# Snowdar/asv-subtools

Hardware: NVIDIA H100
Metric: frames/sec x-vector extraction (80-d fbank) (higher is better)
Workload: dtype f32 (bf16x3 split operands on wgmma, fp32 accumulate in registers)

## Files before the change

asv_subtools_b200/csrc/tdnn_gemm.cu:

```cuda
#include <cuda.h>
#include <cuda_bf16.h>
#include <cuda_runtime.h>

#include <stdlib.h>

#include <mutex>

#include "common.cuh"
#include "ptx.cuh"

namespace xvb {

constexpr int kBlockM = 128;
constexpr int kBlockK = 64;
constexpr int kABytes = kBlockM * kBlockK * 2;
constexpr int kNumConsumers = 256;
constexpr int kProducerWarp = kNumConsumers / 32;
constexpr int kSlabBytes = 16384;
constexpr int kStagePlaneBytes = 64 * kBlockK * 2;
constexpr int kStageOutBytes = 2 * kStagePlaneBytes;
constexpr int kCoefBytes = 3 * kBlockK * 4;
constexpr int kEpiBytes = 2 * (kStageOutBytes + kCoefBytes);
static_assert(kEpiBytes >= kSlabBytes, "the histogram slab lives in the epilogue region");

template <int BLOCK_N, bool kHist, bool kSwish>
__host__ __device__ constexpr bool ping_pong() { return BLOCK_N == 128 && !kHist && !kSwish; }
template <int BLOCK_N, bool kHist, bool kSwish>
__host__ __device__ constexpr int gemm_threads() { return kNumConsumers + (ping_pong<BLOCK_N, kHist, kSwish>() ? 128 : 32); }
constexpr uint32_t kProducerRegs = 40, kConsumerRegs = 232;

struct TdnnGemmParams {
  int B, T, Cin, Cout;
  int Tb, Bb, num_t_blk, num_b_blk, num_n_blk, num_tiles;
  int ntaps, cin_p16, num_cblk;
  int ctx[XVB_MAX_TAPS];
  int flags;
  const float* bias;
  const float* scale;
  const float* shift;
  const float* row_bias;
  const float* utt_bias;
  long long ld_utt;
  int log2_tb;
  float* pool_partial;
  int num_src;
  int unit_first, unit_stride;
  unsigned long long* hist;
  const int* row_label;
  const int* col_label;
  float hist_lo, hist_inv_w;
  int hist_bins;
  int hist_sym;
  int hist_group, num_units;
  int k_slices, kb_per_slice;
  int group_ng, group_kg;
  int out_T;
  const int* lengths;
  int tma_store;
#ifdef XVB_TILE_TIMELINE
  unsigned long long* timeline;
  int timeline_tiles;
  int timeline_general;
#endif
  __nv_bfloat16* y_hi;
  __nv_bfloat16* y_lo;
  long long ldy;
  float* y_f32;
  long long ldyf;
};

template <int BLOCK_N, bool kPool, bool kHist>
__host__ __device__ constexpr bool staged_epilogue() { return !kPool && !kHist && BLOCK_N % kBlockK == 0; }

template <int BLOCK_N, bool kPool, bool kHist>
struct GemmCfg {
  static constexpr int kTailBytes = (staged_epilogue<BLOCK_N, kPool, kHist>() || kPool) ? kEpiBytes : kSlabBytes;
  static constexpr int kBBytes = BLOCK_N * kBlockK * 2;
  static constexpr int kStageBytes = 2 * kABytes + 2 * kBBytes;
  static constexpr int kStages = (192 * 1024) / kStageBytes > 6 ? 6 : (192 * 1024) / kStageBytes;
  static constexpr int kAccRegs = BLOCK_N / 2;
  static constexpr int kSmemBytes = kStages * kStageBytes + kTailBytes + 1024  + 256 ;
  static_assert(kSmemBytes <= 232448, "exceeds the 227 KB shared memory of an sm_90 CTA");
  static_assert(kStages >= 2, "need at least a double-buffered operand pipeline");
};

template <bool kHist>
__device__ __forceinline__ bool decode_tile(const TdnnGemmParams& p, int tile, int& m_unit, int& n_blk, int& slice) {
  slice = 0;
  if constexpr (!kHist) {
    if (p.k_slices > 1) { slice = tile % p.k_slices; tile /= p.k_slices; }
    m_unit = p.unit_first + (tile / p.num_n_blk) * p.unit_stride;
    n_blk = tile % p.num_n_blk;
    return true;
  } else {
    const int per_band = p.num_n_blk * p.hist_group;
    const int band = tile / per_band, r = tile - band * per_band;
    n_blk = r / p.hist_group;
    const int mi = band * p.hist_group + (r - n_blk * p.hist_group);
    m_unit = 2 * (p.unit_first + (mi >> 1) * p.unit_stride) + (mi & 1);
    return mi < 2 * p.num_units && !(p.hist_sym && n_blk < m_unit);
  }
}

__device__ __forceinline__ void chan_merge(float& n, float& mean, float& m2, float nb, float meanb, float m2b) {
  const float tot = n + nb;
  if (tot > 0.f) {
    const float d = meanb - mean, wb = nb / tot;
    mean = fmaf(d, wb, mean);
    m2 += m2b + d * d * n * wb;
  }
  n = tot;
}

__device__ __noinline__ float epi_tanh(float v) { return tanhf(v); }
__device__ __noinline__ float epi_sigmoid(float v) { return 1.f / (1.f + expf(-v)); }

__device__ __noinline__ void epi_zero_row(const TdnnGemmParams& p, long long grow, long long frow, int c_begin, int c_end) {
  for (int c = c_begin; c < c_end; c += 8) {
    const bool has1 = c + 1 < p.Cout;
    if (p.y_hi) {
      if (has1) {
        *reinterpret_cast<uint32_t*>(p.y_hi + grow * p.ldy + c) = 0u;
        *reinterpret_cast<uint32_t*>(p.y_lo + grow * p.ldy + c) = 0u;
      } else {
        p.y_hi[grow * p.ldy + c] = __float2bfloat16(0.f);
        p.y_lo[grow * p.ldy + c] = __float2bfloat16(0.f);
      }
    }
    if (p.y_f32) {
      float* df = p.y_f32 + frow * p.ldyf + c;
      if (has1) *reinterpret_cast<float2*>(df) = make_float2(0.f, 0.f);
      else *df = 0.f;
    }
  }
}

#ifdef XVB_TILE_TIMELINE
#define XVB_TL(...) __VA_ARGS__
constexpr int kTimelineHead = 8, kTimelineRec = 12;
static unsigned long long* g_timeline = nullptr;
static int g_timeline_tiles = 0;
static bool g_timeline_direct = false;
__device__ __forceinline__ unsigned long long global_timer() {
  unsigned long long t;
  asm volatile("mov.u64 %0, %%globaltimer;" : "=l"(t));
  return t;
}
#else
#define XVB_TL(...)
#endif

template <int BLOCK_N, bool kPool, bool kHist, bool kSwish = false>
__global__ void __launch_bounds__(gemm_threads<BLOCK_N, kHist, kSwish>(), 1)
tdnn_gemm_bf16x3_kernel(const __grid_constant__ CUtensorMap map_a_hi, const __grid_constant__ CUtensorMap map_a_lo,
                        const __grid_constant__ CUtensorMap map_a2_hi, const __grid_constant__ CUtensorMap map_a2_lo,
                        const __grid_constant__ CUtensorMap map_w_hi, const __grid_constant__ CUtensorMap map_w_lo,
                        const __grid_constant__ CUtensorMap map_y_hi, const __grid_constant__ CUtensorMap map_y_lo,
                        const __grid_constant__ TdnnGemmParams p) {
  constexpr bool kStaged = staged_epilogue<BLOCK_N, kPool, kHist>();
  using Cfg = GemmCfg<BLOCK_N, kPool, kHist>;
  constexpr int kStages = Cfg::kStages;
  constexpr int kBBytes = Cfg::kBBytes;
  constexpr int kStageBytes = Cfg::kStageBytes;
  static_assert(!kPool || BLOCK_N == kBlockM, "fused pooling: 128 channels x 128 frames per tile");
  constexpr bool kPingPong = ping_pong<BLOCK_N, kHist, kSwish>();
  constexpr int kHalves = kPingPong ? 2 : 1;
  constexpr int kReleaseWarps = kPingPong ? 4 : kNumConsumers / 32;

  extern __shared__ uint8_t smem_raw[];
  uint8_t* smem = reinterpret_cast<uint8_t*>((reinterpret_cast<uintptr_t>(smem_raw) + 1023) & ~uintptr_t(1023));
  uint8_t* slab_base = smem + kStages * kStageBytes;
  uint64_t* full_bar = reinterpret_cast<uint64_t*>(slab_base + Cfg::kTailBytes);
  uint64_t* empty_bar = full_bar + kStages;

  const int warp = threadIdx.x >> 5;
  const int lane = threadIdx.x & 31;

  if (warp == kProducerWarp && lane == 0) {
    tma_prefetch_desc(&map_a_hi);
    tma_prefetch_desc(&map_a_lo);
    tma_prefetch_desc(&map_w_hi);
    tma_prefetch_desc(&map_w_lo);
    if ((kStaged || kPool) && p.tma_store) {
      tma_prefetch_desc(&map_y_hi);
      tma_prefetch_desc(&map_y_lo);
    }
    for (int i = 0; i < kStages; ++i) {
      mbar_init(&full_bar[i], 1);
      mbar_init(&empty_bar[i], kReleaseWarps);
    }
    fence_barrier_init();
  }
  __syncthreads();
  asm volatile("griddepcontrol.wait;" ::: "memory");
  asm volatile("fence.proxy.async;" ::: "memory");

  const int num_kblk = p.num_src * p.ntaps * p.num_cblk;

  if (warp >= kProducerWarp) {
    if constexpr (kPingPong) setmaxnreg_dec<kProducerRegs>();
    if (warp == kProducerWarp && lane == 0) {
      int stage = 0;
      uint32_t phase = 0;
      for (int tile = blockIdx.x; tile < p.num_tiles; tile += gridDim.x) {
        int m_unit, n_blk, slice;
        if (!decode_tile<kHist>(p, tile, m_unit, n_blk, slice)) continue;
        const int cb_begin = slice * p.kb_per_slice;
        const int cb_end = p.k_slices > 1 ? min(p.num_cblk, cb_begin + p.kb_per_slice) : p.num_cblk;
        const int b0 = (m_unit / p.num_t_blk) * p.Bb, t0 = (m_unit % p.num_t_blk) * p.Tb;
        const int n0 = n_blk * BLOCK_N;
        const int a_c0 = p.group_ng ? (n0 / p.group_ng) * p.group_kg : 0;
        for (int src = 0; src < p.num_src; ++src) {
          const CUtensorMap* ma_hi = src == 0 ? &map_a_hi : &map_a2_hi;
          const CUtensorMap* ma_lo = src == 0 ? &map_a_lo : &map_a2_lo;
          for (int tap = 0; tap < p.ntaps; ++tap) {
            const int tt = t0 + p.ctx[tap];
            for (int cb = cb_begin; cb < cb_end; ++cb) {
              mbar_wait(&empty_bar[stage], phase ^ 1);
              uint8_t* s = smem + stage * kStageBytes;
              const int kw = tap * p.cin_p16 + cb * kBlockK;
              mbar_expect_tx(&full_bar[stage], kStageBytes);
              tma_load_3d(s, ma_hi, &full_bar[stage], a_c0 + cb * kBlockK, tt, b0);
              tma_load_3d(s + kABytes, ma_lo, &full_bar[stage], a_c0 + cb * kBlockK, tt, b0);
              tma_load_2d(s + 2 * kABytes, &map_w_hi, &full_bar[stage], kw, n0);
              tma_load_2d(s + 2 * kABytes + kBBytes, &map_w_lo, &full_bar[stage], kw, n0);
              if (++stage == kStages) { stage = 0; phase ^= 1; }
            }
          }
        }
      }
    }
    return;
  }

  if constexpr (kPingPong) setmaxnreg_inc<kConsumerRegs>();
  const int wg = warp >> 2;
  const int q4 = lane & 3;
  const int row_base = kPingPong ? 0 : 64 * wg;
  const int row0 = row_base + 16 * (warp & 3) + (lane >> 2);
  const int etid = threadIdx.x;
  const bool relu = (p.flags & XVB_RELU) != 0;
  const bool bn = (p.flags & XVB_BN) != 0;
  const bool act_sigmoid = (p.flags & XVB_SIGMOID) != 0;
  const bool act_tanh = (p.flags & XVB_TANH) != 0;
  const float relu_floor = relu ? 0.f : -INFINITY;
  float acc[kHalves][Cfg::kAccRegs];
#pragma unroll
  for (int hh = 0; hh < kHalves; ++hh)
#pragma unroll
    for (int i = 0; i < Cfg::kAccRegs; ++i) acc[hh][i] = 0.f;
  auto half_down = [&]() {
#pragma unroll
    for (int i = 0; i < Cfg::kAccRegs; ++i) acc[0][i] = acc[kHalves - 1][i];
  };
  int stage = 0;
  uint32_t phase = 0;
  uint32_t it = 0;

  uint32_t h_below[2] = {0u, 0u}, h_above[2] = {0u, 0u};
  const uint32_t hslab = smem_u32(slab_base);
  auto hist_flush = [&]() {
    asm volatile("bar.sync 1, 256;" ::: "memory");
#pragma unroll
    for (int c = 0; c < 2; ++c) {
      if (h_below[c]) asm volatile("red.shared.add.u32 [%0], %1;" ::"r"(hslab + (c * p.hist_bins) * 4), "r"(h_below[c]) : "memory");
      if (h_above[c]) asm volatile("red.shared.add.u32 [%0], %1;" ::"r"(hslab + (c * p.hist_bins + p.hist_bins - 1) * 4), "r"(h_above[c]) : "memory");
      h_below[c] = 0u; h_above[c] = 0u;
    }
    asm volatile("bar.sync 1, 256;" ::: "memory");
    for (int e = etid; e < 2 * p.hist_bins; e += kNumConsumers) {
      uint32_t c;
      asm volatile("ld.shared.u32 %0, [%1];" : "=r"(c) : "r"(hslab + e * 4) : "memory");
      if (c) {
        atomicAdd(p.hist + e, (unsigned long long)c);
        asm volatile("st.shared.u32 [%0], %1;" ::"r"(hslab + e * 4), "r"(0u) : "memory");
      }
    }
    asm volatile("bar.sync 1, 256;" ::: "memory");
  };
  if constexpr (kHist) {
    for (int e = etid; e < 2 * p.hist_bins; e += kNumConsumers)
      asm volatile("st.shared.u32 [%0], %1;" ::"r"(hslab + e * 4), "r"(0u) : "memory");
    asm volatile("bar.sync 1, 256;" ::: "memory");
  }

  XVB_TL(
    long long tl_start = 0, tl_first = 0, tl_issued = 0, tl_retired = 0, tl_wait = 0;
    long long tl_ep[4] = {0, 0, 0, 0};
    long long tl_t = 0;
    auto tl_mark = [&](int ph) { const long long t = clock64(); tl_ep[ph] += t - tl_t; tl_t = t; };
    unsigned long long* tl_cta = p.timeline ? p.timeline + (size_t)blockIdx.x * (kTimelineHead + (size_t)kTimelineRec * p.timeline_tiles) : nullptr;
    if (tl_cta && threadIdx.x == 0) { tl_cta[0] = global_timer(); tl_cta[1] = (unsigned long long)clock64(); }
  )
  int tj = 0;
  XVB_TL(auto tl_flush = [&]() {
    if (tl_cta && (threadIdx.x & 127) == 0 && tj < p.timeline_tiles) {
      unsigned long long* r = tl_cta + kTimelineHead + (size_t)kTimelineRec * tj;
      r[0] = (unsigned long long)tl_start; r[1] = (unsigned long long)tl_first; r[2] = (unsigned long long)tl_issued;
      r[3] = (unsigned long long)tl_retired; r[4] = (unsigned long long)clock64(); r[5] = (unsigned long long)tl_wait;
      r[6] = (unsigned long long)wg; r[7] = 1ull;
      for (int ph = 0; ph < 4; ++ph) r[8 + ph] = (unsigned long long)tl_ep[ph];
    }
  };)
  for (int tile = blockIdx.x; tile < p.num_tiles; tile += gridDim.x, ++tj) {
    int m_unit, n_blk, slice;
    if (!decode_tile<kHist>(p, tile, m_unit, n_blk, slice)) continue;
    int kb_begin = 0, kb_end = num_kblk;
    if (p.k_slices > 1) {
      kb_begin = slice * p.kb_per_slice;
      kb_end = min(num_kblk, kb_begin + p.kb_per_slice);
    }
    if constexpr (kPingPong) {
      if ((tj & 1) != wg) {
        stage += kb_end - kb_begin;
        phase ^= (uint32_t)(stage / kStages) & 1u;
        stage %= kStages;
        continue;
      }
      if (tj > 0) {
        if (kPool && (threadIdx.x & 127) == 0) tma_store_wait_read<0>();
        asm volatile("bar.sync %0, 256;" ::"r"(2 + wg) : "memory");
      }
    }
    ++it;
    XVB_TL(tl_start = clock64(); tl_wait = 0; tl_ep[0] = tl_ep[1] = tl_ep[2] = tl_ep[3] = 0;)
    auto stage_before = [&]() { return stage == 0 ? kStages - 1 : stage - 1; };
    for (int kb = kb_begin; kb < kb_end; ++kb) {
      XVB_TL(const long long tl_w0 = clock64();)
      mbar_wait(&full_bar[stage], phase);
      XVB_TL(const long long tl_w1 = clock64(); tl_wait += tl_w1 - tl_w0; tl_first = kb == kb_begin ? tl_w1 : tl_first;)
      const uint32_t sa = smem_u32(smem + stage * kStageBytes);
      const uint64_t dx_hi = make_sw128_desc(sa), dx_lo = make_sw128_desc(sa + kABytes);
      const uint64_t dw_hi = make_sw128_desc(sa + 2 * kABytes), dw_lo = make_sw128_desc(sa + 2 * kABytes + kBBytes);
      const uint64_t da_hi = kPool ? dw_hi : dx_hi, da_lo = kPool ? dw_lo : dx_lo;
      const uint64_t db_hi = kPool ? dx_hi : dw_hi, db_lo = kPool ? dx_lo : dw_lo;
      wgmma_fence();
#pragma unroll
      for (int s = 0; s < kBlockK / 16; ++s) {
        const uint64_t koff = (uint64_t)(s * 32 >> 4);
#pragma unroll
        for (int hh = 0; hh < kHalves; ++hh) {
          const uint64_t m_off = (uint64_t)((row_base + 64 * hh) * 128 >> 4);
          wgmma_bf16<BLOCK_N>(acc[hh], da_lo + m_off + koff, db_hi + koff, s == 0 ? (uint32_t)(kb != kb_begin) : 1u);
          wgmma_bf16<BLOCK_N>(acc[hh], da_hi + m_off + koff, db_lo + koff, 1);
          wgmma_bf16<BLOCK_N>(acc[hh], da_hi + m_off + koff, db_hi + koff, 1);
        }
      }
      wgmma_commit();
      wgmma_wait<1>();
      if (kb != kb_begin && lane == 0) mbar_arrive(&empty_bar[stage_before()]);
      if (++stage == kStages) { stage = 0; phase ^= 1; }
    }
    if (kPingPong && tile + gridDim.x < p.num_tiles) asm volatile("bar.arrive %0, 256;" ::"r"(3 - wg) : "memory");
    XVB_TL(tl_issued = clock64();)
    wgmma_wait<0>();
    XVB_TL(tl_retired = clock64(); tl_t = tl_retired;)
#pragma unroll
    for (int hh = 0; hh < kHalves; ++hh) wgmma_fence_operands(acc[hh]);
    if (kb_end > kb_begin && lane == 0) mbar_arrive(&empty_bar[stage_before()]);

    const int b0 = (m_unit / p.num_t_blk) * p.Bb, t0 = (m_unit % p.num_t_blk) * p.Tb;
    const int n0 = n_blk * BLOCK_N;

    if constexpr (kPool) {
      int nv = p.T - t0;
      nv = nv < 0 ? 0 : (nv > p.Tb ? p.Tb : nv);
      const int tblk = m_unit % p.num_t_blk;
      const int gl = p.Tb < 8 ? p.Tb : 8;
#pragma unroll 1
      for (int hh = 0; hh < kHalves; ++hh) {
      if (hh > 0) half_down();
      int b0h = b0, nvh = nv;
      asm volatile("" : "+r"(b0h), "+r"(nvh));
      if (p.tma_store && p.Tb == 8 && nvh == 8 XVB_TL(&& !p.timeline_general)) {
#pragma unroll
        for (int h = 0; h < 2; ++h) {
          const int cch = n0 + row0 + 64 * hh + 8 * h;
          const bool cvalid = cch < p.Cout;
          const float bias_c = (cvalid && p.bias) ? __ldg(p.bias + cch) : 0.f;
          const float scale_c = (cvalid && bn) ? __ldg(p.scale + cch) : 1.f;
          const float shift_c = (cvalid && bn) ? __ldg(p.shift + cch) : 0.f;
          int tid = threadIdx.x;
          asm volatile("" : "+r"(tid));
          const uint32_t dst0 = smem_u32(slab_base) + (tid >> 7) * kStageOutBytes +
                                4 * (16 * ((tid >> 5) & 3) + ((tid & 31) >> 2) + 64 * hh + 8 * h);
#pragma unroll
          for (int i = 0; i < BLOCK_N / 8; ++i) {
            const float x0 = fmaf(fmaxf(acc[0][4 * i + 2 * h] + bias_c, relu_floor), scale_c, shift_c);
            const float x1 = fmaf(fmaxf(acc[0][4 * i + 2 * h + 1] + bias_c, relu_floor), scale_c, shift_c);
            float mean = 0.5f * (x0 + x1) + 0.f;
            float m2 = 0.5f * (x0 - x1) * (x0 - x1);
            float d = __shfl_xor_sync(0xffffffffu, mean, 1) - mean;
            float m2b = __shfl_xor_sync(0xffffffffu, m2, 1);
            mean = fmaf(d, 0.5f, mean);
            m2 += m2b + d * d * 2.f * 0.5f;
            d = __shfl_xor_sync(0xffffffffu, mean, 2) - mean;
            m2b = __shfl_xor_sync(0xffffffffu, m2, 2);
            mean = fmaf(d, 0.5f, mean);
            m2 += m2b + d * d * 4.f * 0.5f;
            if (q4 == 0) {
              st_shared_f32(dst0 + 2 * 4 * BLOCK_N * i, mean);
              st_shared_f32(dst0 + 2 * 4 * BLOCK_N * i + 4 * BLOCK_N, m2);
            }
          }
        }
        XVB_TL(tl_mark(2);)
        continue;
      }
#pragma unroll
      for (int h = 0; h < 2; ++h) {
        const int cch = n0 + row0 + 64 * hh + 8 * h;
        const bool cvalid = cch < p.Cout;
        const float bias_c = (cvalid && p.bias) ? __ldg(p.bias + cch) : 0.f;
        const float scale_c = (cvalid && bn) ? __ldg(p.scale + cch) : 1.f;
        const float shift_c = (cvalid && bn) ? __ldg(p.shift + cch) : 0.f;
        auto emit = [&](int col, float mean, float m2) {
          const int bb = b0h + (col >> p.log2_tb);
          if (cvalid && bb < p.B) {
            float* dst = p.pool_partial + ((long long)tblk * p.B + bb) * (2LL * p.Cout) + cch;
            dst[0] = mean;
            dst[p.Cout] = m2;
          }
        };
        float rn = 0.f, rmean = 0.f, rm2 = 0.f;
#pragma unroll
        for (int i = 0; i < BLOCK_N / 8; ++i) {
          const int col = 8 * i + 2 * q4;
          const float x0 = fmaf(fmaxf(acc[0][4 * i + 2 * h] + bias_c, relu_floor), scale_c, shift_c);
          const float x1 = fmaf(fmaxf(acc[0][4 * i + 2 * h + 1] + bias_c, relu_floor), scale_c, shift_c);
          if (p.Tb == 1) {
            if (nvh > 0) { emit(col, x0, 0.f); emit(col + 1, x1, 0.f); }
            continue;
          }
          const int j = col & (p.Tb - 1);
          const bool v0 = j < nvh, v1 = j + 1 < nvh;
          const float pn = (float)v0 + (float)v1;
          const float pm = v1 ? 0.5f * (x0 + x1) : (v0 ? x0 : 0.f);
          const float pm2 = v1 ? 0.5f * (x0 - x1) * (x0 - x1) : 0.f;
          chan_merge(rn, rmean, rm2, pn, pm, pm2);
          if (((col - 2 * q4 + 8) & (p.Tb - 1)) == 0) {
            if (gl >= 4) chan_merge(rn, rmean, rm2, __shfl_xor_sync(0xffffffffu, rn, 1),
                                    __shfl_xor_sync(0xffffffffu, rmean, 1), __shfl_xor_sync(0xffffffffu, rm2, 1));
            if (gl >= 8) chan_merge(rn, rmean, rm2, __shfl_xor_sync(0xffffffffu, rn, 2),
                                    __shfl_xor_sync(0xffffffffu, rmean, 2), __shfl_xor_sync(0xffffffffu, rm2, 2));
            if (((2 * q4) & (gl - 1)) == 0 && rn > 0.f) emit(col & ~(p.Tb - 1), rmean, rm2);
            rn = 0.f; rmean = 0.f; rm2 = 0.f;
          }
        }
      }
      }
      XVB_TL(tl_mark(2);)
      if (p.tma_store && p.Tb == 8 && nv == 8 XVB_TL(&& !p.timeline_general)) {
        fence_proxy_async();
        asm volatile("bar.sync %0, 128;" ::"r"(4 + wg) : "memory");
        XVB_TL(tl_mark(1);)
        if ((threadIdx.x & 127) == 0) {
          tma_store_4d(&map_y_hi, smem_u32(slab_base) + wg * kStageOutBytes, n0, 0, b0, tblk);
          tma_store_commit();
        }
        XVB_TL(tl_mark(3);)
      }
      XVB_TL(tl_flush();)
      continue;
    }

    if constexpr (kHist) {
      const float top = (float)(p.hist_bins - 2);
#pragma unroll
      for (int h = 0; h < 2; ++h) {
        const int row = row0 + 8 * h;
        const int b = b0 + (row >> p.log2_tb), t = t0 + (row & (p.Tb - 1));
        const bool valid = (b < p.B) && (t < p.T);
        const float rbias = (p.row_bias && valid) ? __ldg(p.row_bias + (long long)b * p.T + t) : 0.f;
        const int lab_r = valid ? __ldg(p.row_label + b) : -1;
#pragma unroll
        for (int i = 0; i < BLOCK_N / 8; ++i) {
#pragma unroll
          for (int e = 0; e < 2; ++e) {
            const int c = n0 + 8 * i + 2 * q4 + e;
            const bool in = c < p.Cout;
            const uint32_t ok = (valid && in && (!p.hist_sym || c > b)) ? 1u : 0u;
            const float sc = acc[0][4 * i + 2 * h + e] + ((in && p.bias) ? __ldg(p.bias + c) : 0.f) + rbias;
            const float x = (sc - p.hist_lo) * p.hist_inv_w;
            const uint32_t cls = (in && __ldg(p.col_label + c) == lab_r) ? 1u : 0u;
            const uint32_t bl = x < 0.f ? ok : 0u;
            const uint32_t ab = !(x < top) ? ok : 0u;
            h_below[0] += bl & (cls ^ 1u); h_below[1] += bl & cls;
            h_above[0] += ab & (cls ^ 1u); h_above[1] += ab & cls;
            if (ok & ~(bl | ab))
              asm volatile("red.shared.add.u32 [%0], %1;" ::"r"(hslab + ((int)cls * p.hist_bins + 1 + (int)x) * 4), "r"(1u) : "memory");
          }
        }
      }
      if ((it & 0x3fffu) == 0) hist_flush();
      continue;
    }

    if constexpr (kStaged) {
      if (p.tma_store) {
        int tid = threadIdx.x;
        asm volatile("" : "+r"(tid));
        const int wgo = tid >> 7, wtid = tid & 127, q4o = tid & 3;
        const int prow = 16 * ((tid >> 5) & 3) + ((tid & 31) >> 2);
        const uint32_t stg = smem_u32(slab_base) + wgo * kStageOutBytes;
        const uint32_t coefs = smem_u32(slab_base) + 2 * kStageOutBytes + wgo * kCoefBytes;
        const int ebar = 4 + wgo;
        const uint32_t coef = coefs + 8 * q4o;
        const uint32_t my = stg + (uint32_t)prow * 128u + ((uint32_t)(prow & 7) << 4) + 4u * q4o;
#pragma unroll 1
        for (int hh = 0; hh < kHalves; ++hh) {
          if (hh > 0) half_down();
          const int hrow = (kPingPong ? 0 : 64 * wgo) + 64 * hh;
          uint32_t keep[2];
#pragma unroll
          for (int r = 0; r < 2; ++r) {
            const int row = hrow + prow + 8 * r;
            const int b = b0 + (row >> p.log2_tb), t = t0 + (row & (p.Tb - 1));
            keep[r] = (p.lengths && b < p.B && t >= __ldg(p.lengths + b)) ? 0u : 0xffffffffu;
          }
#pragma unroll
          for (int cr = 0; cr < BLOCK_N / kBlockK; ++cr) {
            const int c0 = n0 + kBlockK * cr;
            if (c0 >= p.Cout) break;
            if (wtid == 0) tma_store_wait_read<0>();
            XVB_TL(tl_mark(0);)
            if (wtid < kBlockK) {
              const int c = c0 + wtid;
              const bool in = c < p.Cout;
              st_shared_f32(coefs + 4 * wtid, (in && p.bias) ? __ldg(p.bias + c) : 0.f);
              st_shared_f32(coefs + 4 * (kBlockK + wtid), (in && bn) ? __ldg(p.scale + c) : 1.f);
              st_shared_f32(coefs + 4 * (2 * kBlockK + wtid), (in && bn) ? __ldg(p.shift + c) : 0.f);
            }
            asm volatile("bar.sync %0, 128;" ::"r"(ebar) : "memory");
            XVB_TL(tl_mark(1);)
#pragma unroll
            for (int i = 0; i < kBlockK / 8; ++i) {
              const float2 bias_c = ld_shared_f2(coef + 32 * i), scale_c = ld_shared_f2(coef + 32 * i + 4 * kBlockK),
                           shift_c = ld_shared_f2(coef + 32 * i + 8 * kBlockK);
              const float bias_e[2] = {bias_c.x, bias_c.y}, scale_e[2] = {scale_c.x, scale_c.y},
                          shift_e[2] = {shift_c.x, shift_c.y};
#pragma unroll
              for (int r = 0; r < 2; ++r) {
                float x[2] = {acc[0][4 * (8 * cr + i) + 2 * r], acc[0][4 * (8 * cr + i) + 2 * r + 1]};
#pragma unroll
                for (int e = 0; e < 2; ++e) {
                  float v = x[e] + bias_e[e] + 0.f;
                  v = fmaxf(v, relu_floor);
                  if constexpr (kSwish) v = v / (1.f + expf(-v));
                  if (bn) v = fmaf(v, scale_e[e], shift_e[e]);
                  if (act_tanh) v = epi_tanh(v);
                  if (act_sigmoid) v = epi_sigmoid(v);
                  x[e] = v;
                }
                __nv_bfloat16 h0, l0, h1, l1;
                split_bf16(x[0], h0, l0);
                split_bf16(x[1], h1, l1);
                const uint32_t at = (my ^ ((uint32_t)i << 4)) + 1024u * r;
                st_shared_u32(at, pack_bf16x2(h0, h1) & keep[r]);
                st_shared_u32(at + kStagePlaneBytes, pack_bf16x2(l0, l1) & keep[r]);
              }
            }
            XVB_TL(tl_mark(2);)
            fence_proxy_async();
            asm volatile("bar.sync %0, 128;" ::"r"(ebar) : "memory");
            if (wtid == 0) {
              const int hb = b0 + (hrow >> p.log2_tb), ht = t0 + (hrow & (p.Tb - 1));
              tma_store_3d(&map_y_hi, stg, c0, ht, hb);
              tma_store_3d(&map_y_lo, stg + kStagePlaneBytes, c0, ht, hb);
              tma_store_commit();
            }
            XVB_TL(tl_mark(3);)
          }
        }
        XVB_TL(tl_flush();)
        continue;
      }
    }
    if constexpr (!kPool && !kHist) {
#pragma unroll 1
      for (int hh = 0; hh < kHalves; ++hh) {
      if (hh > 0) half_down();
      constexpr int kRows = 2;
      bool live[kRows];
      float rbias[kRows];
      const float* ub[kRows];
      long long grow[kRows], frow[kRows];
#pragma unroll
      for (int r = 0; r < kRows; ++r) {
        const int row = row0 + 64 * hh + 8 * r;
        const int b = b0 + (row >> p.log2_tb), t = t0 + (row & (p.Tb - 1));
        live[r] = b < p.B && t < p.T;
        grow[r] = (long long)b * p.T + t;
        frow[r] = (long long)b * p.out_T + t + slice;
        if (live[r] && p.lengths && t >= __ldg(p.lengths + b)) {
          epi_zero_row(p, grow[r], frow[r], n0 + 2 * q4, min(n0 + BLOCK_N, p.Cout));
          live[r] = false;
        }
        rbias[r] = (live[r] && p.row_bias) ? __ldg(p.row_bias + grow[r]) : 0.f;
        ub[r] = (live[r] && p.utt_bias) ? p.utt_bias + (long long)b * p.ld_utt : nullptr;
      }
#pragma unroll
      for (int i = 0; i < BLOCK_N / 8; ++i) {
        const int c = n0 + 8 * i + 2 * q4;
        if (c >= p.Cout) break;
        const bool has1 = c + 1 < p.Cout;
        float bias_c[2], scale_c[2], shift_c[2];
#pragma unroll
        for (int e = 0; e < 2; ++e) {
          const bool in = e == 0 || has1;
          bias_c[e] = (in && p.bias) ? __ldg(p.bias + c + e) : 0.f;
          scale_c[e] = (in && bn) ? __ldg(p.scale + c + e) : 1.f;
          shift_c[e] = (in && bn) ? __ldg(p.shift + c + e) : 0.f;
        }
#pragma unroll
        for (int r = 0; r < kRows; ++r) {
          if (!live[r]) continue;
          float x[2] = {acc[0][4 * i + 2 * r], acc[0][4 * i + 2 * r + 1]};
#pragma unroll
          for (int e = 0; e < 2; ++e) {
            if (e == 1 && !has1) break;
            float v = x[e] + bias_c[e] + rbias[r];
            if (ub[r]) v += __ldg(ub[r] + c + e);
            v = fmaxf(v, relu_floor);
            if constexpr (kSwish) v = v / (1.f + expf(-v));
            if (bn) v = fmaf(v, scale_c[e], shift_c[e]);
            if (act_tanh) v = epi_tanh(v);
            if (act_sigmoid) v = epi_sigmoid(v);
            x[e] = v;
          }
          if (p.y_hi) {
            __nv_bfloat16 h0, l0, h1, l1;
            split_bf16(x[0], h0, l0);
            split_bf16(x[1], h1, l1);
            __nv_bfloat16* dh = p.y_hi + grow[r] * p.ldy + c;
            __nv_bfloat16* dl = p.y_lo + grow[r] * p.ldy + c;
            if (has1) {
              *reinterpret_cast<uint32_t*>(dh) = pack_bf16x2(h0, h1);
              *reinterpret_cast<uint32_t*>(dl) = pack_bf16x2(l0, l1);
            } else {
              *dh = h0;
              *dl = l0;
            }
          }
          if (p.y_f32) {
            float* df = p.y_f32 + frow[r] * p.ldyf + c;
            if (has1) *reinterpret_cast<float2*>(df) = make_float2(x[0], x[1]);
            else *df = x[0];
          }
        }
      }
      }
      XVB_TL(tl_flush();)
    }
  }
  if constexpr (kHist) hist_flush();
  if constexpr (kStaged || kPool) {
    if (p.tma_store && (threadIdx.x & 127) == 0) tma_store_wait_done<0>();
  }
  XVB_TL(if (tl_cta && (threadIdx.x & 127) == 0) { tl_cta[2 + 2 * wg] = global_timer(); tl_cta[3 + 2 * wg] = (unsigned long long)clock64(); })
}

__global__ void segment_reduce_kernel(const float* __restrict__ part, int S, int B, int Cout, const float* __restrict__ bias,
                                      const float* __restrict__ scale, const float* __restrict__ shift, int flags,
                                      float* __restrict__ y_f32, long long ldyf, __nv_bfloat16* __restrict__ y_hi,
                                      __nv_bfloat16* __restrict__ y_lo, long long ldy) {
  asm volatile("griddepcontrol.wait;" ::: "memory");
  const long long idx = blockIdx.x * (long long)blockDim.x + threadIdx.x;
  if (idx >= (long long)B * Cout) return;
  const int b = (int)(idx / Cout), c = (int)(idx - (long long)b * Cout);
  const float* src = part + (long long)b * S * Cout + c;
  float x = src[0];
  for (int s = 1; s < S; ++s) x += src[(long long)s * Cout];
  x += bias ? bias[c] : 0.f;
  if (flags & XVB_RELU) x = fmaxf(x, 0.f);
  if (flags & XVB_BN) x = fmaf(x, scale[c], shift[c]);
  if (flags & XVB_TANH) x = tanhf(x);
  if (flags & XVB_SIGMOID) x = 1.f / (1.f + expf(-x));
  if (y_f32) y_f32[(long long)b * ldyf + c] = x;
  if (y_hi) {
    __nv_bfloat16 h, l;
    split_bf16(x, h, l);
    y_hi[(long long)b * ldy + c] = h;
    y_lo[(long long)b * ldy + c] = l;
  }
}

typedef CUresult (*PFN_encodeTiled)(CUtensorMap*, CUtensorMapDataType, cuuint32_t, void*, const cuuint64_t*,
                                    const cuuint64_t*, const cuuint32_t*, const cuuint32_t*, CUtensorMapInterleave,
                                    CUtensorMapSwizzle, CUtensorMapL2promotion, CUtensorMapFloatOOBfill);

static PFN_encodeTiled get_encode() {
  static PFN_encodeTiled fn = nullptr;
  static std::once_flag once;
  std::call_once(once, [] {
    void* p = nullptr;
    cudaDriverEntryPointQueryResult q;
    if (cudaGetDriverEntryPoint("cuTensorMapEncodeTiled", &p, cudaEnableDefault, &q) == cudaSuccess &&
        q == cudaDriverEntryPointSuccess)
      fn = reinterpret_cast<PFN_encodeTiled>(p);
  });
  return fn;
}

int make_tensor_map(CUtensorMap* m, const void* base, int esize, int rank, const unsigned long long* dims,
                    const unsigned long long* strides_bytes, const unsigned* box, int swizzle_bytes) {
  PFN_encodeTiled enc = get_encode();
  if (!enc) { set_error("cuTensorMapEncodeTiled entry point not available"); return XVB_ECUDA; }
  cuuint64_t d[5], st[4];
  cuuint32_t bx[5], es[5];
  for (int i = 0; i < rank; ++i) { d[i] = dims[i]; bx[i] = box[i]; es[i] = 1; }
  for (int i = 0; i + 1 < rank; ++i) st[i] = strides_bytes[i];
  const CUtensorMapSwizzle sw = swizzle_bytes == 128 ? CU_TENSOR_MAP_SWIZZLE_128B
                               : swizzle_bytes == 64 ? CU_TENSOR_MAP_SWIZZLE_64B : CU_TENSOR_MAP_SWIZZLE_NONE;
  CUresult r = enc(m, esize == 2 ? CU_TENSOR_MAP_DATA_TYPE_BFLOAT16 : CU_TENSOR_MAP_DATA_TYPE_FLOAT32, rank,
                   const_cast<void*>(base), d, st, bx, es, CU_TENSOR_MAP_INTERLEAVE_NONE, sw,
                   CU_TENSOR_MAP_L2_PROMOTION_L2_256B, CU_TENSOR_MAP_FLOAT_OOB_FILL_NONE);
  if (r != CUDA_SUCCESS) { set_error("cuTensorMapEncodeTiled(rank %d) failed: %d", rank, (int)r); return XVB_ECUDA; }
  return XVB_OK;
}

static int make_frame_map(CUtensorMap* m, const void* base, int C, int T, int B, long long ld, int Tb, int Bb,
                          long long batch_stride = 0) {
  PFN_encodeTiled enc = get_encode();
  if (!enc) { set_error("cuTensorMapEncodeTiled entry point not available"); return XVB_ECUDA; }
  cuuint64_t dims[3] = {(cuuint64_t)C, (cuuint64_t)T, (cuuint64_t)B};
  cuuint64_t strides[2] = {(cuuint64_t)ld * 2, batch_stride ? (cuuint64_t)batch_stride * 2 : (cuuint64_t)ld * 2 * (cuuint64_t)T};
  cuuint32_t box[3] = {(cuuint32_t)kBlockK, (cuuint32_t)Tb, (cuuint32_t)Bb};
  cuuint32_t estr[3] = {1, 1, 1};
  CUresult r = enc(m, CU_TENSOR_MAP_DATA_TYPE_BFLOAT16, 3, const_cast<void*>(base), dims, strides, box, estr,
                   CU_TENSOR_MAP_INTERLEAVE_NONE, CU_TENSOR_MAP_SWIZZLE_128B, CU_TENSOR_MAP_L2_PROMOTION_L2_256B,
                   CU_TENSOR_MAP_FLOAT_OOB_FILL_NONE);
  if (r != CUDA_SUCCESS) { set_error("cuTensorMapEncodeTiled(frame map C=%d T=%d B=%d ld=%lld) failed: %d", C, T, B, ld, (int)r); return XVB_ECUDA; }
  return XVB_OK;
}

static int make_store_map(CUtensorMap* m, const void* base, int Cout, int T, int B, long long ld, int Tb) {
  const int box_t = Tb < 64 ? Tb : 64;
  const unsigned long long dims[3] = {(unsigned long long)Cout, (unsigned long long)T, (unsigned long long)B};
  const unsigned long long strides[2] = {(unsigned long long)ld * 2, (unsigned long long)ld * 2 * (unsigned long long)T};
  const unsigned box[3] = {(unsigned)kBlockK, (unsigned)box_t, (unsigned)(64 / box_t)};
  return make_tensor_map(m, base, 2, 3, dims, strides, box, 128);
}

static int make_partial_map(CUtensorMap* m, const float* base, int Cout, int B, int nblk) {
  const unsigned long long dims[4] = {(unsigned long long)Cout, 2ull, (unsigned long long)B, (unsigned long long)nblk};
  const unsigned long long strides[3] = {4ull * Cout, 8ull * Cout, 8ull * Cout * (unsigned long long)B};
  const unsigned box[4] = {(unsigned)kBlockM, 2u, 16u, 1u};
  return make_tensor_map(m, base, 4, 4, dims, strides, box, 0);
}

static int make_weight_map(CUtensorMap* m, const void* base, long long K, int Cout, int block_n) {
  PFN_encodeTiled enc = get_encode();
  if (!enc) { set_error("cuTensorMapEncodeTiled entry point not available"); return XVB_ECUDA; }
  cuuint64_t dims[2] = {(cuuint64_t)K, (cuuint64_t)Cout};
  cuuint64_t strides[1] = {(cuuint64_t)K * 2};
  cuuint32_t box[2] = {(cuuint32_t)kBlockK, (cuuint32_t)block_n};
  cuuint32_t estr[2] = {1, 1};
  CUresult r = enc(m, CU_TENSOR_MAP_DATA_TYPE_BFLOAT16, 2, const_cast<void*>(base), dims, strides, box, estr,
                   CU_TENSOR_MAP_INTERLEAVE_NONE, CU_TENSOR_MAP_SWIZZLE_128B, CU_TENSOR_MAP_L2_PROMOTION_L2_256B,
                   CU_TENSOR_MAP_FLOAT_OOB_FILL_NONE);
  if (r != CUDA_SUCCESS) { set_error("cuTensorMapEncodeTiled(weight map K=%lld Cout=%d) failed: %d", K, Cout, (int)r); return XVB_ECUDA; }
  return XVB_OK;
}

static void choose_m_tile(int B, int T, int* Tb_out, int* Bb_out, int max_tb = 128) {
  if (T == 1) {
    *Tb_out = 1;
    *Bb_out = 128;
    return;
  }
  long long best = -1;
  int bt = max_tb;
  for (int Tb = max_tb; Tb >= 1; Tb >>= 1) {
    const int Bb = 128 / Tb;
    const long long rows = (long long)((T + Tb - 1) / Tb) * Tb * ((B + Bb - 1) / Bb) * Bb;
    if (best < 0 || rows < best) { best = rows; bt = Tb; }
  }
  *Tb_out = bt;
  *Bb_out = 128 / bt;
}

struct GemmPlan {
  CUtensorMap ma_hi, ma_lo, ma2_hi, ma2_lo, mw_hi, mw_lo, my_hi, my_lo;
  TdnnGemmParams p;
  int (*launch)(const GemmPlan&, const TdnnGemmParams&, cudaStream_t) = nullptr;
  int grid = 0;
  int pdl = 1;
  bool reduce = false;
  const float* r_bias = nullptr; const float* r_scale = nullptr; const float* r_shift = nullptr;
  int r_flags = 0;
  float* r_y_f32 = nullptr; long long r_ldyf = 0;
  __nv_bfloat16* r_y_hi = nullptr; __nv_bfloat16* r_y_lo = nullptr; long long r_ldy = 0;
};

template <int BLOCK_N, bool kPool, bool kHist, bool kSwish>
static int launch_inst(const GemmPlan& pl, const TdnnGemmParams& p, cudaStream_t stream) {
  using Cfg = GemmCfg<BLOCK_N, kPool, kHist>;
  XVB_ENSURE_DYN_SMEM((tdnn_gemm_bf16x3_kernel<BLOCK_N, kPool, kHist, kSwish>), Cfg::kSmemBytes);
  cudaLaunchConfig_t cfg{};
  cfg.gridDim = dim3(pl.grid);
  cfg.blockDim = dim3(gemm_threads<BLOCK_N, kHist, kSwish>());
  cfg.dynamicSmemBytes = Cfg::kSmemBytes;
  cfg.stream = stream;
  cudaLaunchAttribute attr[1];
  attr[0].id = cudaLaunchAttributeProgrammaticStreamSerialization;
  attr[0].val.programmaticStreamSerializationAllowed = 1;
  cfg.attrs = attr;
  cfg.numAttrs = pl.pdl ? 1 : 0;
  XVB_CUDA(cudaLaunchKernelEx(&cfg, tdnn_gemm_bf16x3_kernel<BLOCK_N, kPool, kHist, kSwish>, pl.ma_hi, pl.ma_lo, pl.ma2_hi,
                              pl.ma2_lo, pl.mw_hi, pl.mw_lo, pl.my_hi, pl.my_lo, p));
  XVB_LAUNCH_CHECK();
  return XVB_OK;
}

template <int BLOCK_N, bool kPool = false, bool kHist = false, bool kSwish = false>
static int prepare_gemm(GemmPlan& pl, const void* w_hi, const void* w_lo) {
  TdnnGemmParams& p = pl.p;
  const long long K = (long long)p.ntaps * p.cin_p16;
  int rc = make_weight_map(&pl.mw_hi, w_hi, K, p.Cout, BLOCK_N);
  if (rc) return rc;
  rc = make_weight_map(&pl.mw_lo, w_lo, K, p.Cout, BLOCK_N);
  if (rc) return rc;
  p.num_n_blk = (p.Cout + BLOCK_N - 1) / BLOCK_N;
  p.tma_store = staged_epilogue<BLOCK_N, kPool, kHist>() && p.y_hi && !p.y_f32 && p.k_slices == 1 && !p.row_bias && !p.utt_bias &&
                p.Cout % 8 == 0;
  if (kPool) p.tma_store = p.Tb == 8;
  XVB_TL(if (g_timeline_direct) p.tma_store = 0;)
  if (kPool && p.tma_store) {
    if ((rc = make_partial_map(&pl.my_hi, p.pool_partial, p.Cout, p.B, p.num_t_blk))) return rc;
    pl.my_lo = pl.mw_lo;
  } else if (p.tma_store) {
    if ((rc = make_store_map(&pl.my_hi, p.y_hi, p.Cout, p.T, p.B, p.ldy, p.Tb))) return rc;
    if ((rc = make_store_map(&pl.my_lo, p.y_lo, p.Cout, p.T, p.B, p.ldy, p.Tb))) return rc;
  } else {
    pl.my_hi = pl.mw_hi; pl.my_lo = pl.mw_lo;
  }
  const int all_m_units = kHist ? (p.num_t_blk * p.num_b_blk + 1) / 2 : p.num_t_blk * p.num_b_blk;
  if (p.unit_first >= all_m_units) { pl.launch = nullptr; return XVB_OK; }
  const int num_m_units = (all_m_units - p.unit_first + p.unit_stride - 1) / p.unit_stride;
  p.num_units = num_m_units;
  p.hist_group = 8;
  const long long tiles = kHist ? (long long)((2 * num_m_units + p.hist_group - 1) / p.hist_group) * p.hist_group * p.num_n_blk
                                : (long long)num_m_units * p.num_n_blk * (p.k_slices > 1 ? p.k_slices : 1);
  XVB_CHECK_ARG(tiles < (1ll << 31), "xvb_tdnn_affine: %d x %d tiles exceed one launch", num_m_units, p.num_n_blk);
  p.num_tiles = (int)tiles;
  p.out_T = p.k_slices > 1 ? p.k_slices : p.T;
  const int sms = sm_count();
  pl.grid = p.num_tiles < sms ? p.num_tiles : sms;
  static const int pdl = getenv("XVB_PDL") ? atoi(getenv("XVB_PDL")) : 1;
  pl.pdl = pdl;
  pl.launch = &launch_inst<BLOCK_N, kPool, kHist, kSwish>;
  return XVB_OK;
}

static int splitk_slices(const xvb_tdnn_args_t& a, bool has_hist, int* kb_per_slice) {
  const int num_cblk = (a.Cin + kBlockK - 1) / kBlockK;
  *kb_per_slice = num_cblk;
  const int splitk = getenv("XVB_SPLITK") ? atoi(getenv("XVB_SPLITK")) : 1;
  if (!(splitk && a.T == 1 && a.ntaps == 1 && !a.x2_hi && !a.pool_partial && !has_hist && !a.row_bias && !a.utt_bias &&
        !(a.flags & XVB_SWISH) && a.groups <= 1 &&
        a.B <= 1024 && num_cblk >= 24 && a.Cout % 4 == 0))
    return 1;
  int S = num_cblk / 6;
  S = S > 8 ? 8 : S;
  *kb_per_slice = (num_cblk + S - 1) / S;
  return (num_cblk + *kb_per_slice - 1) / *kb_per_slice;
}

}

using namespace xvb;

size_t xvb::gemm_plan_scratch_bytes(const xvb_tdnn_args_t& a, const TrialHist* th) {
  int kb;
  const int S = splitk_slices(a, th != nullptr, &kb);
  return S > 1 ? (size_t)a.B * S * a.Cout * sizeof(float) : 0;
}

int xvb::gemm_plan_build(GemmPlan** out, const xvb_tdnn_args_t& a, const TrialHist* th, void* scratch) {
  int rc = require_sm90();
  if (rc) return rc;
  *out = nullptr;
  const int B = a.B, T = a.T, Cin = a.Cin, Cout = a.Cout, ntaps = a.ntaps;
  XVB_CHECK_ARG(a.x_hi && a.x_lo && a.w_hi && a.w_lo, "xvb_tdnn_affine: null operand pointer");
  XVB_CHECK_ARG(B > 0 && T > 0 && Cin > 0 && Cout > 0, "xvb_tdnn_affine: bad shape B=%d T=%d Cin=%d Cout=%d", B, T, Cin, Cout);
  XVB_CHECK_ARG(ntaps >= 1 && ntaps <= XVB_MAX_TAPS && a.context_host, "xvb_tdnn_affine: ntaps=%d out of range", ntaps);
  if (a.x_batch_stride)
    XVB_CHECK_ARG(a.ldx % 8 == 0 && a.x_batch_stride % 8 == 0 && !a.x2_hi && ntaps == 1 &&
                  a.x_batch_stride >= (long long)(T - 1) * a.ldx + Cin,
                  "xvb_tdnn_affine: x_batch_stride=%lld needs ntaps==1, no second source, 8-element alignment and room for T windows",
                  (long long)a.x_batch_stride);
  else
    XVB_CHECK_ARG(a.ldx % 8 == 0 && a.ldx >= Cin, "xvb_tdnn_affine: ldx=%lld must be a multiple of 8 and >= Cin", (long long)a.ldx);
  XVB_CHECK_ARG((a.x2_hi != nullptr) == (a.x2_lo != nullptr), "xvb_tdnn_affine: x2_hi/x2_lo must both be set or both NULL");
  if (a.x2_hi) XVB_CHECK_ARG(a.ldx2 % 8 == 0 && a.ldx2 >= Cin, "xvb_tdnn_affine: ldx2=%lld must be a multiple of 8 and >= Cin", (long long)a.ldx2);
  XVB_CHECK_ARG((a.y_hi != nullptr) == (a.y_lo != nullptr), "xvb_tdnn_affine: y_hi/y_lo must both be set or both NULL");
  XVB_CHECK_ARG(a.y_hi || a.y_f32 || a.pool_partial || th, "xvb_tdnn_affine: no output requested");
  XVB_CHECK_ARG(!(a.flags & XVB_SWISH) || !(a.pool_partial || th), "xvb_tdnn_affine: XVB_SWISH is a layer-epilogue flag only");
  XVB_CHECK_ARG(!(a.lengths && (th || a.pool_partial)), "xvb_tdnn_affine: lengths apply to the layer epilogue only");
  if (a.pool_partial) XVB_CHECK_ARG(!a.y_hi && !a.y_f32 && Cout % 4 == 0 && (uintptr_t)a.pool_partial % 16 == 0,
                                    "xvb_tdnn_affine: pool_partial excludes other outputs and needs Cout%%4==0");
  if (a.y_hi) XVB_CHECK_ARG(a.ldy % 8 == 0 && a.ldy >= Cout, "xvb_tdnn_affine: plane output needs ldy%%8==0 and ldy>=Cout");
  if (a.y_f32) XVB_CHECK_ARG(a.ldyf % 4 == 0 && a.ldyf >= Cout, "xvb_tdnn_affine: fp32 output needs ldyf%%4==0 and ldyf>=Cout");
  XVB_CHECK_ARG(!(a.flags & XVB_BN) || (a.bn_scale && a.bn_shift), "xvb_tdnn_affine: XVB_BN without scale/shift");
  if (a.utt_bias) XVB_CHECK_ARG(a.ld_utt_bias % 4 == 0 && a.ld_utt_bias >= Cout && Cout % 4 == 0 && (uintptr_t)a.utt_bias % 16 == 0,
                                "xvb_tdnn_affine: utt_bias needs ld%%4==0, Cout%%4==0, 16-byte alignment");
  XVB_CHECK_ARG(((uintptr_t)a.x_hi | (uintptr_t)a.x_lo | (uintptr_t)a.x2_hi | (uintptr_t)a.x2_lo | (uintptr_t)a.w_hi |
                 (uintptr_t)a.w_lo | (uintptr_t)a.y_hi | (uintptr_t)a.y_lo | (uintptr_t)a.y_f32) % 16 == 0,
                "xvb_tdnn_affine: pointers must be 16-byte aligned");
  for (int i = 1; i < ntaps; ++i)
    XVB_CHECK_ARG(a.context_host[i] > a.context_host[i - 1], "xvb_tdnn_affine: context must be strictly increasing (components.py:34-36)");
  const int G = a.groups > 1 ? a.groups : 1;
  if (G > 1)
    XVB_CHECK_ARG(xvb_tdnn_grouped_fits(Cin, Cout, G) && ntaps == 1 && !a.x2_hi && !a.pool_partial && !th && !a.x_batch_stride &&
                  !(a.flags & XVB_SWISH),
                  "xvb_tdnn_affine: groups=%d needs Cin/groups %% 64 == 0, Cout/groups %% 32 == 0, one tap and no second source, "
                  "fused pooling, histogram, im2col view or XVB_SWISH (Cin=%d Cout=%d ntaps=%d)", G, Cin, Cout, ntaps);

  GemmPlan* plp = new GemmPlan();
  struct Guard { GemmPlan* p; ~Guard() { delete p; } } guard{plp};
  GemmPlan& pl = *plp;
  TdnnGemmParams& p = pl.p;
  p = TdnnGemmParams{};
  p.B = B; p.T = T; p.Cin = Cin; p.Cout = Cout;
  choose_m_tile(B, T, &p.Tb, &p.Bb);
  p.num_t_blk = (T + p.Tb - 1) / p.Tb;
  p.num_b_blk = (B + p.Bb - 1) / p.Bb;
  p.ntaps = ntaps;
  p.cin_p16 = (int)round_up(Cin / G, 16);
  p.num_cblk = (Cin / G + kBlockK - 1) / kBlockK;
  if (G > 1) { p.group_ng = Cout / G; p.group_kg = Cin / G; }
  for (int i = 0; i < ntaps; ++i) p.ctx[i] = a.context_host[i];
  p.flags = a.flags;
  p.bias = a.bias; p.scale = a.bn_scale; p.shift = a.bn_shift; p.row_bias = a.row_bias;
  p.utt_bias = a.utt_bias; p.ld_utt = a.ld_utt_bias;
  p.pool_partial = a.pool_partial;
  p.lengths = a.lengths;
  p.num_src = a.x2_hi ? 2 : 1;
  p.unit_first = 0; p.unit_stride = 1;
  if (th) {
    p.hist = th->hist; p.row_label = th->row_label; p.col_label = th->col_label;
    p.hist_lo = th->lo; p.hist_inv_w = th->inv_w; p.hist_bins = th->nbins; p.hist_sym = th->symmetric;
    p.unit_first = th->unit_first; p.unit_stride = th->unit_stride;
  }
  p.log2_tb = 0;
  while ((1 << p.log2_tb) < p.Tb) ++p.log2_tb;
  p.y_hi = reinterpret_cast<__nv_bfloat16*>(a.y_hi);
  p.y_lo = reinterpret_cast<__nv_bfloat16*>(a.y_lo);
  p.ldy = a.ldy; p.y_f32 = a.y_f32; p.ldyf = a.ldyf;

  XVB_TL(p.timeline = g_timeline; p.timeline_tiles = g_timeline_tiles; p.timeline_general = g_timeline_direct;)
// ... 137 lines not shown
```

Measured before the change: 34.99 million.

## Cut consumer register pressure via smem parking, branchless epilogue, and specialized activations

Several unrelated micro-changes to the TDNN wgmma GEMM kernel. Ping-pong consumers park their loop state (stage, phase, tile, tj) in shared memory and reload it, and re-decode the tile after the mainloop, so fewer registers stay live across the accumulator region. The direct-store epilogue becomes branchless: masked predicated stores with 32-bit row indices replace the noinline zero-row helper and early breaks. The staged epilogue gets a compile-time variant without tanh/sigmoid, and chan_merge uses an rcp-plus-double-Newton division. The aim is to avoid spills and branch overhead, at the cost of extra smem traffic, int32 index overflow risk, and harder-to-follow code.

```diff
diff --git a/asv_subtools_b200/csrc/tdnn_gemm.cu b/asv_subtools_b200/csrc/tdnn_gemm.cu
--- a/asv_subtools_b200/csrc/tdnn_gemm.cu
+++ b/asv_subtools_b200/csrc/tdnn_gemm.cu
@@ -5,6 +5,7 @@
 #include <stdlib.h>
 
 #include <mutex>
+#include <type_traits>
 
 #include "common.cuh"
 #include "ptx.cuh"
@@ -102,10 +103,18 @@
   }
 }
 
+__device__ __forceinline__ float count_ratio(float nb, float tot) {
+  float r;
+  asm("rcp.approx.ftz.f32 %0, %1;" : "=f"(r) : "f"(tot));
+  const double d = (double)tot, y = (double)r;
+  const double y1 = fma(y, fma(-d, y, 1.0), y);
+  return __double2float_rn((double)nb * y1);
+}
+
 __device__ __forceinline__ void chan_merge(float& n, float& mean, float& m2, float nb, float meanb, float m2b) {
   const float tot = n + nb;
   if (tot > 0.f) {
-    const float d = meanb - mean, wb = nb / tot;
+    const float d = meanb - mean, wb = count_ratio(nb, tot);
     mean = fmaf(d, wb, mean);
     m2 += m2b + d * d * n * wb;
   }
@@ -114,26 +123,6 @@
 
 __device__ __noinline__ float epi_tanh(float v) { return tanhf(v); }
 __device__ __noinline__ float epi_sigmoid(float v) { return 1.f / (1.f + expf(-v)); }
-
-__device__ __noinline__ void epi_zero_row(const TdnnGemmParams& p, long long grow, long long frow, int c_begin, int c_end) {
-  for (int c = c_begin; c < c_end; c += 8) {
-    const bool has1 = c + 1 < p.Cout;
-    if (p.y_hi) {
-      if (has1) {
-        *reinterpret_cast<uint32_t*>(p.y_hi + grow * p.ldy + c) = 0u;
-        *reinterpret_cast<uint32_t*>(p.y_lo + grow * p.ldy + c) = 0u;
-      } else {
-        p.y_hi[grow * p.ldy + c] = __float2bfloat16(0.f);
-        p.y_lo[grow * p.ldy + c] = __float2bfloat16(0.f);
-      }
-    }
-    if (p.y_f32) {
-      float* df = p.y_f32 + frow * p.ldyf + c;
-      if (has1) *reinterpret_cast<float2*>(df) = make_float2(0.f, 0.f);
-      else *df = 0.f;
-    }
-  }
-}
 
 #ifdef XVB_TILE_TIMELINE
 #define XVB_TL(...) __VA_ARGS__
@@ -243,6 +232,7 @@
   const bool bn = (p.flags & XVB_BN) != 0;
   const bool act_sigmoid = (p.flags & XVB_SIGMOID) != 0;
   const bool act_tanh = (p.flags & XVB_TANH) != 0;
+  const bool act = act_tanh || act_sigmoid;
   const float relu_floor = relu ? 0.f : -INFINITY;
   float acc[kHalves][Cfg::kAccRegs];
 #pragma unroll
@@ -302,7 +292,18 @@
       for (int ph = 0; ph < 4; ++ph) r[8 + ph] = (unsigned long long)tl_ep[ph];
     }
   };)
-  for (int tile = blockIdx.x; tile < p.num_tiles; tile += gridDim.x, ++tj) {
+  int tile = blockIdx.x;
+  const uint32_t park_slot = smem_u32(empty_bar + kStages) + 16u * (uint32_t)warp;
+  auto park = [&]() {
+    if constexpr (kPingPong) st_shared_v4(park_slot, (uint32_t)stage, phase, (uint32_t)tile, (uint32_t)tj);
+  };
+  auto unpark = [&]() {
+    if constexpr (kPingPong) {
+      const uint4 st = ld_shared_u4(park_slot);
+      stage = (int)st.x; phase = st.y; tile = (int)st.z; tj = (int)st.w;
+    }
+  };
+  for (; tile < p.num_tiles; unpark(), tile += gridDim.x, ++tj) {
     int m_unit, n_blk, slice;
     if (!decode_tile<kHist>(p, tile, m_unit, n_blk, slice)) continue;
     int kb_begin = 0, kb_end = num_kblk;
@@ -315,6 +316,7 @@
         stage += kb_end - kb_begin;
         phase ^= (uint32_t)(stage / kStages) & 1u;
         stage %= kStages;
+        park();
         continue;
       }
       if (tj > 0) {
@@ -325,11 +327,13 @@
     ++it;
     XVB_TL(tl_start = clock64(); tl_wait = 0; tl_ep[0] = tl_ep[1] = tl_ep[2] = tl_ep[3] = 0;)
     auto stage_before = [&]() { return stage == 0 ? kStages - 1 : stage - 1; };
+    uint32_t ring = smem_u32(smem);
+    asm volatile("" : "+r"(ring));
     for (int kb = kb_begin; kb < kb_end; ++kb) {
       XVB_TL(const long long tl_w0 = clock64();)
       mbar_wait(&full_bar[stage], phase);
       XVB_TL(const long long tl_w1 = clock64(); tl_wait += tl_w1 - tl_w0; tl_first = kb == kb_begin ? tl_w1 : tl_first;)
-      const uint32_t sa = smem_u32(smem + stage * kStageBytes);
+      const uint32_t sa = ring + (uint32_t)(stage * kStageBytes);
       const uint64_t dx_hi = make_sw128_desc(sa), dx_lo = make_sw128_desc(sa + kABytes);
       const uint64_t dw_hi = make_sw128_desc(sa + 2 * kABytes), dw_lo = make_sw128_desc(sa + 2 * kABytes + kBBytes);
       const uint64_t da_hi = kPool ? dw_hi : dx_hi, da_lo = kPool ? dw_lo : dx_lo;
@@ -358,6 +362,8 @@
 #pragma unroll
     for (int hh = 0; hh < kHalves; ++hh) wgmma_fence_operands(acc[hh]);
     if (kb_end > kb_begin && lane == 0) mbar_arrive(&empty_bar[stage_before()]);
+    if constexpr (kPingPong) decode_tile<kHist>(p, tile, m_unit, n_blk, slice);
+    park();
 
     const int b0 = (m_unit / p.num_t_blk) * p.Bb, t0 = (m_unit % p.num_t_blk) * p.Tb;
     const int n0 = n_blk * BLOCK_N;
@@ -533,6 +539,7 @@
             }
             asm volatile("bar.sync %0, 128;" ::"r"(ebar) : "memory");
             XVB_TL(tl_mark(1);)
+            auto stage_values = [&](auto with_act) {
 #pragma unroll
             for (int i = 0; i < kBlockK / 8; ++i) {
               const float2 bias_c = ld_shared_f2(coef + 32 * i), scale_c = ld_shared_f2(coef + 32 * i + 4 * kBlockK),
@@ -548,8 +555,10 @@
                   v = fmaxf(v, relu_floor);
                   if constexpr (kSwish) v = v / (1.f + expf(-v));
                   if (bn) v = fmaf(v, scale_e[e], shift_e[e]);
-                  if (act_tanh) v = epi_tanh(v);
-                  if (act_sigmoid) v = epi_sigmoid(v);
+                  if constexpr (decltype(with_act)::value) {
+                    if (act_tanh) v = epi_tanh(v);
+                    if (act_sigmoid) v = epi_sigmoid(v);
+                  }
                   x[e] = v;
                 }
                 __nv_bfloat16 h0, l0, h1, l1;
@@ -560,6 +569,9 @@
                 st_shared_u32(at + kStagePlaneBytes, pack_bf16x2(l0, l1) & keep[r]);
               }
             }
+            };
+            if (!kPingPong || act) stage_values(std::true_type{});
+            else stage_values(std::false_type{});
             XVB_TL(tl_mark(2);)
             fence_proxy_async();
             asm volatile("bar.sync %0, 128;" ::"r"(ebar) : "memory");
@@ -582,45 +594,42 @@
       if (hh > 0) half_down();
       constexpr int kRows = 2;
       bool live[kRows];
+      uint32_t keep[kRows];
       float rbias[kRows];
-      const float* ub[kRows];
-      long long grow[kRows], frow[kRows];
+      int urow[kRows], grow[kRows], frow[kRows];
 #pragma unroll
       for (int r = 0; r < kRows; ++r) {
         const int row = row0 + 64 * hh + 8 * r;
         const int b = b0 + (row >> p.log2_tb), t = t0 + (row & (p.Tb - 1));
         live[r] = b < p.B && t < p.T;
-        grow[r] = (long long)b * p.T + t;
-        frow[r] = (long long)b * p.out_T + t + slice;
-        if (live[r] && p.lengths && t >= __ldg(p.lengths + b)) {
-          epi_zero_row(p, grow[r], frow[r], n0 + 2 * q4, min(n0 + BLOCK_N, p.Cout));
-          live[r] = false;
-        }
+        grow[r] = b * p.T + t;
+        frow[r] = b * p.out_T + t + slice;
+        keep[r] = (live[r] && p.lengths && t >= __ldg(p.lengths + b)) ? 0u : 0xffffffffu;
         rbias[r] = (live[r] && p.row_bias) ? __ldg(p.row_bias + grow[r]) : 0.f;
-        ub[r] = (live[r] && p.utt_bias) ? p.utt_bias + (long long)b * p.ld_utt : nullptr;
-      }
+        urow[r] = (live[r] && p.utt_bias) ? b : -1;
+      }
+      const bool out_hi = p.y_hi != nullptr, out_f32 = p.y_f32 != nullptr;
 #pragma unroll
       for (int i = 0; i < BLOCK_N / 8; ++i) {
         const int c = n0 + 8 * i + 2 * q4;
-        if (c >= p.Cout) break;
-        const bool has1 = c + 1 < p.Cout;
+        const bool has0 = c < p.Cout, has1 = c + 1 < p.Cout;
         float bias_c[2], scale_c[2], shift_c[2];
 #pragma unroll
         for (int e = 0; e < 2; ++e) {
-          const bool in = e == 0 || has1;
-          bias_c[e] = (in && p.bias) ? __ldg(p.bias + c + e) : 0.f;
-          scale_c[e] = (in && bn) ? __ldg(p.scale + c + e) : 1.f;
-          shift_c[e] = (in && bn) ? __ldg(p.shift + c + e) : 0.f;
+          const bool in = e == 0 ? has0 : has1;
+          bias_c[e] = (in && p.bias) ? p.bias[c + e] : 0.f;
+          scale_c[e] = (in && bn) ? p.scale[c + e] : 1.f;
+          shift_c[e] = (in && bn) ? p.shift[c + e] : 0.f;
         }
 #pragma unroll
         for (int r = 0; r < kRows; ++r) {
-          if (!live[r]) continue;
           float x[2] = {acc[0][4 * i + 2 * r], acc[0][4 * i + 2 * r + 1]};
 #pragma unroll
           for (int e = 0; e < 2; ++e) {
-            if (e == 1 && !has1) break;
             float v = x[e] + bias_c[e] + rbias[r];
-            if (ub[r]) v += __ldg(ub[r] + c + e);
+            const bool has_u = urow[r] >= 0 && (e == 0 ? has0 : has1);
+            const float u = has_u ? p.utt_bias[(long long)urow[r] * p.ld_utt + c + e] : 0.f;
+            v = has_u ? v + u : v;
             v = fmaxf(v, relu_floor);
             if constexpr (kSwish) v = v / (1.f + expf(-v));
             if (bn) v = fmaf(v, scale_c[e], shift_c[e]);
@@ -628,25 +637,20 @@
             if (act_sigmoid) v = epi_sigmoid(v);
             x[e] = v;
           }
-          if (p.y_hi) {
-            __nv_bfloat16 h0, l0, h1, l1;
-            split_bf16(x[0], h0, l0);
-            split_bf16(x[1], h1, l1);
-            __nv_bfloat16* dh = p.y_hi + grow[r] * p.ldy + c;
-            __nv_bfloat16* dl = p.y_lo + grow[r] * p.ldy + c;
-            if (has1) {
-              *reinterpret_cast<uint32_t*>(dh) = pack_bf16x2(h0, h1);
-              *reinterpret_cast<uint32_t*>(dl) = pack_bf16x2(l0, l1);
-            } else {
-              *dh = h0;
-              *dl = l0;
-            }
-          }
-          if (p.y_f32) {
-            float* df = p.y_f32 + frow[r] * p.ldyf + c;
-            if (has1) *reinterpret_cast<float2*>(df) = make_float2(x[0], x[1]);
-            else *df = x[0];
-          }
+          const bool st2 = live[r] && has1, st1 = live[r] && has0 && !has1;
+          __nv_bfloat16 h0, l0, h1, l1;
+          split_bf16(x[0], h0, l0);
+          split_bf16(x[1], h1, l1);
+          const uint32_t hw = pack_bf16x2(h0, h1) & keep[r], lw = pack_bf16x2(l0, l1) & keep[r];
+          const long long o = (long long)grow[r] * p.ldy + c;
+          if (out_hi && st2) *reinterpret_cast<uint32_t*>(p.y_hi + o) = hw;
+          if (out_hi && st2) *reinterpret_cast<uint32_t*>(p.y_lo + o) = lw;
+          if (out_hi && st1) *reinterpret_cast<uint16_t*>(p.y_hi + o) = (uint16_t)hw;
+          if (out_hi && st1) *reinterpret_cast<uint16_t*>(p.y_lo + o) = (uint16_t)lw;
+          float* df = p.y_f32 + (long long)frow[r] * p.ldyf + c;
+          const float f0 = keep[r] ? x[0] : 0.f, f1 = keep[r] ? x[1] : 0.f;
+          if (out_f32 && st2) *reinterpret_cast<float2*>(df) = make_float2(f0, f1);
+          if (out_f32 && st1) *df = f0;
         }
       }
       }
```

Result: faster. 35.86 million (median of 6 runs) (+2.5%).
